# ufcg-lsd/custom-k8s-scheduler

Hardware: AMD Instinct MI355X
Metric: pods scheduled/sec (exact sequential stream, 5,000 nodes x 100,000 pods) (higher is better)
Workload: dtype int32+f64; 1 GPU; config2: 5,000 nodes x 100,000 pods, exact sequential, Fit+Balanced+QoS weights, percentageOfNodesToScore=100; engine=lookahead, launch=resident, table_layout=compact, lookahead=32, parallelism=single

## Files before the change

### custom-k8s-scheduler_amd/csrc/qs_ctx.hpp

```cpp
#pragma once
#include <hip/hip_runtime.h>
#include <rccl/rccl.h>

#include <mutex>
#include <string>
#include <unordered_map>
#include <vector>

#include "../../include/qsched.h"
#include "qs_device.hpp"
#include "qs_launch.hpp"

namespace qs_host {

constexpr int64_t kLimit = (1LL << 24) - 1;
constexpr int64_t kWideMemLimit = (1LL << 46) - 1;
constexpr int64_t kGrowLimit32 = (1LL << 31) - 1;
constexpr int64_t kGrowLimitF64 = (1LL << 53) - 1;
constexpr uint32_t kSoaMinNodes = 1u << 16;
constexpr uint32_t kAaMaxNodes = 1u << 20;

struct QsError {
    qs_status st;
    std::string msg;
// ... 97 lines not shown
    uint64_t epoch_after = 0;
    bool aa_ran = false;
    int32_t spread_row[qs::kMaxZones];
    uint32_t spread_apps = 0;
    std::vector<uint8_t> soft;
    std::vector<uint8_t> hosts;
    uint32_t host_pods = 0;
    int32_t host_row[16];
    uint32_t host_apps = 0;
    int shift = 0;
    bool wide = false;
    std::vector<uint32_t> run0;
    std::vector<uint32_t> uni_bits;
    qs_host::DevBuf d_uni;
    uint32_t uni_K = 0, uni_count = 0, uni_given = 0;
    qs_ctx *owner = nullptr;
    hipGraphExec_t gexec = nullptr;
    std::vector<uint8_t> gkey;
    ~qs_stream() {
        if (gexec) (void)hipGraphExecDestroy(gexec);
    }
};

struct qs_ctx {
    std::mutex mu;
    uint64_t table_epoch = 0;
    qs_config cfg{};
    int device = 0;
    hipStream_t stream = nullptr;
    hipStream_t stream2 = nullptr;
// ... 100 lines not shown
```

### custom-k8s-scheduler_amd/csrc/qs_host.cpp

```cpp
#include "../../include/qsched.h"

#include <hip/hip_runtime.h>

#include <algorithm>
#include <atomic>
#include <chrono>
#include <cmath>
#include <cstddef>
#include <cstdio>
#include <cstdlib>
#include <cstring>
#include <exception>
#include <mutex>
#include <new>
#include <string>
#include <vector>
#include <functional>
#include <condition_variable>
#include <thread>

#include "qs_ctx.hpp"

using namespace qs;

// ... 23 lines not shown
        const char d = env_char("QS_RES_DIAG");
        return d == '1' || d == '2';
    }();
};
const ProcKnobs &proc_knobs() {
    static const ProcKnobs k;
    return k;
}

struct RunKnobs {
    bool norm_waves1 = env_is("QS_NORM_WAVES", '1');
    bool resident_off = env_is("QS_RESIDENT", '0');
    bool res_k32_off = env_is("QS_RES_K32", '0');
    bool fast_alloc_off = env_is("QS_FAST_ALLOC", '0');
    bool res_uniform_off = env_is("QS_RES_UNIFORM", '0');
    bool fused_merge_off = env_is("QS_BATCH_FUSED_MERGE", '0');
    const char *inject = getenv("QS_INJECT_FAULT");
    bool hosttime = getenv("QS_HOSTTIME") != nullptr;
    bool norm_diag = getenv("QS_NORM_DIAG") != nullptr;
    bool sel_diag = env_is("QS_RES_DIAG", '1');
};

uint32_t feat_of(const qs_config &c) {
    uint32_t f = 0;
    if (c.enable_taint) f |= kFeatTaint;
    if (c.enable_affinity) f |= kFeatAffinity;
    return f;
}

void check_cfg(const qs_config &c) {
// ... 1216 lines not shown
            if (s->run0[last] <= s0) {
                s->uni_bits[w >> 5] |= 1u << (w & 31);
                ++s->uni_count;
            }
        }
        s->d_uni.ensure(4 * s->uni_bits.size());
        HIPCHK(hipMemcpyAsync(s->d_uni.p, s->uni_bits.data(), 4 * s->uni_bits.size(),
                              hipMemcpyHostToDevice, c->stream));
        s->uni_K = K;
    }
    if (!s->uni_count) return nullptr;
    s->uni_given = s->uni_count;
    return s->d_uni.as<uint32_t>();
}

void la_report_res_diag(const uint64_t *h, uint32_t sel) {
    const double nw = h[3] ? (double)h[3] : 1.0;
    fprintf(stderr, "QS_RES_DIAG resolver %.3f us per window; windows whose lists were not prefetched %llu of %llu (selectors %u)\n",
            h[1] * 0.01 / nw, (unsigned long long)h[4], (unsigned long long)h[3], sel);
    if (h[2])
        fprintf(stderr, "QS_RES_DIAG selector 0: done seen %.2f us, its task finished %.2f us after "
                        "the resolver's start of the window it overlaps (%llu windows)\n",
                h[13] * 0.01 / (double)h[2], h[14] * 0.01 / (double)h[2], (unsigned long long)h[2]);
    {
        std::vector<double> fin;
        for (uint32_t k = 0; k < std::min(sel, 64u); ++k)
            if (h[64 + k]) fin.push_back(h[64 + k] * 0.01);
        std::sort(fin.begin(), fin.end());
        if (!fin.empty()) {
            fprintf(stderr, "QS_RES_DIAG selectors' mean finish (us after window start), sorted:");
// ... 74 lines not shown
    dcr.inject = (inject_once(c, kn.inject, "resident_stall", kInjResidentStall) ||
                  (kn.inject && std::strcmp(kn.inject, "resident_stall_always") == 0)) ? 1u : 0u;
    if (kn.inject && std::strcmp(kn.inject, "resident_skew") == 0) dcr.inject = 2u;
    dcr.first_ticks = c->world > 1 ? 500000000ull : 0ull;
    dcr.all_alloc = c->zero_alloc == 0 && !kn.fast_alloc_off ? 1u : 0u;
    c->last_res_path = (!r.norm && rgeo.k32 ? 1 : 0) |
                       (!r.norm && !(c->dc.feat & kFeatRes) && dcr.all_alloc ? 2 : 0);
    dcr.sel_diag = kn.sel_diag ? 1u : 0u;
    uint64_t *rdiag = nullptr;
    if (proc_knobs().res_diag) {
        c->diag.ensure(1024);
        rdiag = c->diag.as<uint64_t>();
        HIPCHK(hipMemsetAsync(rdiag, 0, 1024, c->stream));
    }
    const uint32_t *uni = la_uniform_windows(c, s, rgeo, rsh.W, kn);
    kt.begin(3, c->stream);
    HIPCHK(launch_la_stream_res(c->dt, io.dp, io.dx, dcr, r.P, rgeo, c->lists.as<uint64_t>(), c->clists.as<uint64_t>(),
                                (uint32_t)r.lwords, (uint32_t)rcw, c->npart.as<uint4>(),
                                c->normi.as<NormInfo>(), c->nstat.as<uint32_t>(),
                                c->nfall.as<unsigned long long>(), io.on, io.ok,
                                io.st, c->resctl.p, rp.sel, rdiag, rsh, c->stream, uni));
    kt.end(3, c->stream);
    if (rdiag) {
        uint64_t h[128] = {0};
        HIPCHK(hipMemcpyAsync(h, rdiag, 1024, hipMemcpyDeviceToHost, c->stream));
        HIPCHK(hipStreamSynchronize(c->stream));
        la_report_res_diag(h, rp.sel);
    }
}

uint64_t run_lookahead(qs_ctx *c, qs_stream *s, const RunIo &io, const RunKnobs &kn, KernelTimer &kt) {
    const ProcKnobs &pk = proc_knobs();
    const LaRun r = la_setup(c, s, io, kn, kt.on);
    const auto th0 = std::chrono::steady_clock::now();
    const bool graph_ok = !c->comm || pk.graph == '1';
    const bool use_graph = graph_ok && !r.handoff && !r.mbox && !kt.on && !pk.diag && pk.graph != '0';
// ... 80 lines not shown
        }
        stats->pods = P;
        stats->evals = (uint64_t)P * n;
        stats->wall_s = ms * 1e-3;
        stats->batches = batches;
        stats->truncations = rescans;
        stats->engine_used = eng;
        stats->table_layout = c->wide ? 1 : 0;
        stats->resumed_windows = resumed;
        stats->resident = (eng == QS_ENGINE_LOOKAHEAD && c->last_resident) ? 1 : 0;
        stats->resident_path = stats->resident ? c->last_res_path : 0;
        stats->device_faults = c->device_faults;
    }
}

}

extern "C" {

const char *qs_version(void) { return "qsched 0.1 (gfx950)"; }

void qs_config_default(qs_config *cfg) {
    if (!cfg) return;
    std::memset(cfg, 0, sizeof(*cfg));
    cfg->abi_version = QS_ABI_VERSION;
    cfg->engine = QS_ENGINE_AUTO;
    cfg->fit_weight_cpu = 1;
    cfg->fit_weight_mem = 1;
    const int32_t wf[3] = {1, 2, 3}, wb[3] = {1, 1, 1};
    for (int q = 0; q < 3; q++) { cfg->w_fit[q] = wf[q]; cfg->w_bal[q] = wb[q]; }
// ... 693 lines not shown
            const uint32_t j = s->order[k];
            s->soft[k] = pod_soft_spread(pods[j]) ? 1 : 0;
            s->hosts[k] = pod_host_spread(pods[j]) ? 1 : 0;
            s->host_pods += s->hosts[k];
            if (s->hosts[k] && !host_seen[(uint32_t)pods[j].app]) {
                host_seen[(uint32_t)pods[j].app] = 1;
                if (s->host_apps < kHostSpreadApps) s->host_row[s->host_apps] = pods[j].app;
                ++s->host_apps;
            }
            compact_pod(c, pods[j], j, c->shift, c->wide, dp.data() + rb * k);
            if (needx) dx[k] = compact_podx(c, pods[j]);
        }
        s->run0.resize(p);
        for (uint32_t k = 0; k < p; k++)
            s->run0[k] = k > 0 && std::memcmp(dp.data() + rb * k, dp.data() + rb * (k - 1), rb) == 0 ? s->run0[k - 1] : k;
        const size_t P1 = std::max<uint32_t>(p, 1);
        s->d_pods.ensure(rb * P1);
        s->d_podx.ensure(sizeof(DPodX) * dx.size());
        s->d_node.ensure(4 * P1);
        s->d_key.ensure(8 * P1);
        if (c->cfg.record_timestamps) s->d_stamp.ensure(8 * P1);
        HIPCHK(hipMemcpyAsync(s->d_pods.p, dp.data(), rb * p, hipMemcpyHostToDevice, c->stream));
        HIPCHK(hipMemcpyAsync(s->d_podx.p, dx.data(), sizeof(DPodX) * dx.size(), hipMemcpyHostToDevice, c->stream));
        HIPCHK(hipStreamSynchronize(c->stream));
        c->streams.push_back(s);
        s->owner = c;
    });
    if (st != QS_OK) {
        delete s;
        return st;
// ... 2 lines not shown
    return QS_OK;
}

qs_status qs_stream_run(qs_ctx *c, qs_stream *s, qs_mode mode, qs_stats *stats) {
    return guarded(c, [&] {
        if (!s) fail(QS_EINVAL, "null stream");
        if (mode != QS_MODE_EXACT && mode != QS_MODE_BATCHED) fail(QS_EINVAL, "unknown qs_mode");
        if (s->shift != c->shift || s->wide != c->wide) fail(QS_ESTATE, "node table re-laid out after prepare");
        if (mode == QS_MODE_BATCHED && (s->spread_apps != 0 || s->host_pods != 0))
            fail(QS_EINVAL, "QS_MODE_BATCHED does not know topology spread (QS_AA_SPREAD / QS_AA_SPREAD_SOFT / QS_AA_SPREAD_HOSTNAME pods, spec S13-S15): "
                            "run the stream in QS_MODE_EXACT on a context that tracks pod anti-affinity");
        HIPCHK(hipSetDevice(c->device));
        s->ran = false;
        s->mode_ran = -1;
        s->uni_given = 0;
        s->aa_ran = false;
        ++c->table_epoch;
        if (!c->dev_valid) upload_table(c);
        const uint32_t n = c->m.n, P = s->p;
        const RunKnobs kn;
        const RunPlan plan = plan_run(c, s, mode);
        if (plan.host_spread && n > 0) ensure_hcount(c);
        if (c->aa_track && !(plan.aa_exact && plan.eng == QS_ENGINE_SCAN)) c->hc_valid = false;
        if (plan.host_spread && plan.eng == QS_ENGINE_PERSISTENT && n > 0 && P > 0)
            HIPCHK(hipMemcpyAsync(c->dt.zcount + (size_t)(kMaxApps + 4) * kMaxZones + 16, s->host_row,
                                  sizeof s->host_row, hipMemcpyHostToDevice, c->stream));
        if (plan.aa_exact && plan.eng == QS_ENGINE_PERSISTENT && n > 0 && P > 0)
            HIPCHK(hipMemcpyAsync(c->dt.zcount + (size_t)(kMaxApps + 1) * kMaxZones, s->spread_row,
                                  sizeof s->spread_row, hipMemcpyHostToDevice, c->stream));
        const RunIo io{s->d_pods.p, s->d_podx.as<DPodX>(), s->d_node.as<int32_t>(), s->d_key.as<uint64_t>(),
// ... 223 lines not shown

qs_status qs_stream_stamps(qs_ctx *c, qs_stream *s, uint64_t *stamps) {
    return guarded(c, [&] {
        if (!s || !s->ran || !s->d_stamp.p) fail(QS_ESTATE, "no timestamps recorded");
        HIPCHK(hipMemcpy(stamps, s->d_stamp.p, 8 * (size_t)s->p, hipMemcpyDeviceToHost));
    });
}

qs_status qs_stream_uniform_windows(qs_ctx *c, qs_stream *s, uint32_t *windows) {
    return guarded(c, [&] {
        if (!s || !windows) fail(QS_EINVAL, "null stream or output");
        *windows = s->ran ? s->uni_given : 0u;
    });
}

}
```

### custom-k8s-scheduler_amd/csrc/qs_kernels.hip

```cpp
#include "qs_kernels.hpp"

namespace qs {

__global__ __launch_bounds__(256) void k_rows_to_soa(DevTable t) {
    const uint32_t i = blockIdx.x * 256 + threadIdx.x;
    if (i >= t.n) return;
    const DRow r = t.rows[i];
    t.soa.c[kSAc][i] = r.ac; t.soa.c[kSAm][i] = r.am; t.soa.c[kSRc][i] = r.rc; t.soa.c[kSRm][i] = r.rm;
    t.soa.c[kSZc][i] = r.zc; t.soa.c[kSZm][i] = r.zm; t.soa.c[kSNp][i] = r.np; t.soa.c[kSMp][i] = r.mp;
    t.soa.c[kSAe0][i] = r.ae0; t.soa.c[kSRe0][i] = r.re0; t.soa.c[kSAe1][i] = r.ae1; t.soa.c[kSRe1][i] = r.re1;
}

__global__ void k_batch_init(uint32_t *ctrl, uint32_t *bidx, uint32_t P, uint32_t B) {
    const uint32_t nb = min(P, B);
    if (threadIdx.x < nb) bidx[threadIdx.x] = threadIdx.x;
    if (threadIdx.x == 0) { ctrl[0] = nb; ctrl[1] = nb; }
}

hipError_t launch_batch_init(uint32_t *ctrl, uint32_t *bidx, uint32_t P, uint32_t B, hipStream_t stream) {
    hipLaunchKernelGGL(k_batch_init, dim3(1), dim3(64), 0, stream, ctrl, bidx, P, B);
    return hipGetLastError();
}

hipError_t batch_claim_prepare() {
// ... 179 lines not shown
                    : (feat & kFeatRes)   ? ((feat & kFeatWide) ? res_wide_la_stream_res_per_cu(geo, feat, n)
                                                              : res_compact_la_stream_res_per_cu(geo, feat, n))
                    : (feat & kFeatWide)  ? wide_la_stream_res_per_cu(geo, feat, n)
                    : (feat & kFeatNorm)  ? la_stream_res_per_cu<kFeatExt | kFeatTaint | kFeatAffinity>(geo, n)
                    : (feat & kFeatExt) ? la_stream_res_per_cu<kFeatExt>(geo, n)
                                        : la_stream_res_per_cu<0>(geo, n);
    const int sgpr_waves = 800 / (((int)kResSgprMax + 15) / 16 * 16 + 16);
    const int safe = std::min(per, sgpr_waves / (kResBS / 64 / 4));
    return (uint32_t)std::max(0, safe) * cus;
}

bool la_stream_res_takes_uniform(const LaGeom &geo, uint32_t feat, uint32_t W) {
    return geo.k32 && W == 1 && geo.K <= 32 && res_uniform_class(feat, geo.E);
}

hipError_t launch_la_stream_res(const DevTable &t, const void *pods, const DPodX *podx, const DevCfg &c, uint32_t P,
                                const LaGeom &geo, uint64_t *lists0, uint64_t *clists0, uint32_t lwords,
                                uint32_t cwords, uint4 *npart, NormInfo *norm, uint32_t *stat, unsigned long long *nfall,
                                int32_t *on, uint64_t *ok, uint64_t *st, void *ctl, uint32_t sel_blocks, uint64_t *rdiag,
                                const ResShard &rsh0, hipStream_t stream, const uint32_t *uni) {
    ResShard rsh = rsh0;
    rsh.uni = la_stream_res_takes_uniform(geo, c.feat, rsh0.W) ? uni : nullptr;
    if (geo.G == 0 || (c.feat & kFeatAA) || (uint64_t)t.n * (t.wrows ? sizeof(DRowW) : sizeof(DRow)) >= (1ull << 31))
        return hipErrorInvalidValue;
    if (c.feat & kFeatStrat)
        return (t.wrows ? strat_wide_la_stream_res : strat_compact_la_stream_res)(
            t, pods, podx, c, P, geo, lists0, clists0, lwords, cwords, npart, norm, stat, nfall, on, ok, st, ctl,
            sel_blocks, rdiag, rsh, stream);
    if (c.feat & kFeatRes)
        return (t.wrows ? res_wide_la_stream_res : res_compact_la_stream_res)(
            t, pods, podx, c, P, geo, lists0, clists0, lwords, cwords, npart, norm, stat, nfall, on, ok, st, ctl,
            sel_blocks, rdiag, rsh, stream);
    if (t.wrows)
        return wide_la_stream_res(t, pods, podx, c, P, geo, lists0, clists0, lwords, cwords, npart, norm, stat, nfall, on,
                                  ok, st, ctl, sel_blocks, rdiag, rsh, stream);
    if (c.feat & kFeatNorm)
        return la_stream_res_f<kFeatExt | kFeatTaint | kFeatAffinity>(t, pods, podx, c, P, geo, lists0, clists0, lwords,
// ... 43 lines not shown
```

### custom-k8s-scheduler_amd/csrc/qs_kernels.hpp

```cpp
#pragma once
#include <algorithm>
#include <cstring>

#include "qs_device.hpp"
#include "qs_launch.hpp"

#ifndef QS_EXP_HOOKS
#define QS_EXP_NORM_AB(norm) (norm)
#define QS_EXP_SLOT_KEY(act, r, q)
#define QS_EXP_CAND_KEY(f, tot, cr, p)
#define QS_EXP_PARK_RETURN()
#endif

#include "qs_key32.hpp"

namespace qs {

constexpr uint32_t kFeatNorm = kFeatTaint | kFeatAffinity;

__device__ __forceinline__ uint64_t *aa_lds_zmask() {
    __shared__ uint64_t zmask[kMaxApps];
    return zmask;
}
template <int N>
// ... 2329 lines not shown
        if (f != tag || (uint32_t)(lo >> 32) != w + 1 || (uint32_t)(hi >> 32) != w + 1) {
            __hip_atomic_store((gu32 *)werr, 1u, __ATOMIC_RELAXED, __HIP_MEMORY_SCOPE_AGENT);
            return false;
        }
        const uint32_t qx = (uint32_t)(lo >> 24) & 0xFFu, qy = (uint32_t)lo & 0xFFFFFFu;
        const uint32_t qz = (uint32_t)(hi >> 22) & 0x3FFu, qw = (uint32_t)hi & 0x3FFFFFu;
        if (qx > nf.mt) { nf.mt = qx; nf.ct = 0; }
        if (qx == nf.mt) nf.ct += qy;
        if (qz > nf.ma) { nf.ma = qz; nf.ca = 0; }
        if (qz == nf.ma) nf.ca += qw;
    }
    out = nf;
    return true;
}

template <int E, int E2, uint32_t F>
__device__ __forceinline__ void res_selector(const DevTable &t, const PodT<F> *__restrict__ pods, const DevCfg &c,
                                             uint32_t P, uint32_t K, uint32_t G, uint32_t L, uint32_t chunk,
                                             uint32_t nwin, uint64_t *lists0, uint64_t *clists0, uint32_t lwords,
                                             uint32_t cwords, ResCtl *ctl, uint32_t sid, uint32_t S,
                                             uint64_t *rdiag, const DPodX *__restrict__ podx, uint4 *npart0,
                                             NormInfo *norm0, uint32_t *stat0, const ResShard &rsh) {
    constexpr bool NORM = (F & kFeatNorm) != 0;
    const uint32_t lo = (uint32_t)((uint64_t)rsh.rank * t.n / rsh.W);
    const uint32_t hi = (uint32_t)((uint64_t)(rsh.rank + 1) * t.n / rsh.W);
    bool hello_ok = rsh.W == 1;
    uint64_t ts0 = 0, ts1 = 0, ts2 = 0, dsc = 0, dtl = 0, dpm = 0, ntask = 0, nmerge = 0;
    uint64_t tdone_ = 0, wstart_ = 0, seen_ = 0, fin_ = 0, nwt_ = 0, lastp_ = 0, nlast_ = 0, late13_ = 0, late15_ = 0;
    __shared__ uint64_t lbuf[64];
    __shared__ uint32_t okflag_[4];
    __shared__ uint32_t nred[4][8];
    uint32_t &okflag = okflag_[0];
    const int tid = threadIdx.x, lane = tid & 63, w8 = tid >> 6;
    const __amdgpu_buffer_rsrc_t rs = row_rsrc<F>(t);
    DevCfg cv = c;
    asm volatile("" : "+v"(cv.yd_both), "+v"(cv.yd_c), "+v"(cv.yd_m), "+v"(cv.wc), "+v"(cv.wm));
    for (uint32_t w = 0; w < nwin; ++w) {
        const uint32_t s0 = w * K, kw = min(K, P - s0), b = w & 1;
        if (sid >= kw * G) continue;
        static_assert(sizeof(PodT<F>) % 16 == 0, "pod record in 16-byte words");
        constexpr int PW = (int)(sizeof(PodT<F>) / 16);
        constexpr bool kPodPre = (F & kFeatNorm) == 0 && E >= 7 && E <= 8;
        u32x4 pq[PW];
        if constexpr (kPodPre) {
            const u32x4 *src = reinterpret_cast<const u32x4 *>(pods + s0 + min(sid / G, kw - 1));
#pragma unroll
            for (int q = 0; q < PW; ++q) pq[q] = src[q];
#pragma unroll
            for (int q = 0; q < PW; ++q) asm volatile("" : "+v"(pq[q]));
        }
        if (w >= 2) {
            if (tid == 0) okflag = res_wait_ge(&ctl->done, w - 1, c.werr) ? 1u : 0u;
            if (rdiag && tid == 0) {
                tdone_ = __builtin_amdgcn_s_memrealtime();
                wstart_ = load_coh_u64(&rdiag[15]);
            }
            __syncthreads();
            if (!okflag) return;
        }
        uint64_t *lists = lists0 + (size_t)b * lwords;
        uint64_t *clists = clists0 + (size_t)b * cwords;
        for (uint32_t task = sid; task < kw * G; task += S) {
            if (c.inject == 1u && w == 3 && task == 0) continue;
            if (c.inject == 2u && w >= 40 && w < 44) {
                if (tid == 0) {
                    const uint64_t t0 = __builtin_amdgcn_s_memrealtime();
                    while (__builtin_amdgcn_s_memrealtime() - t0 < 300000ull) __builtin_amdgcn_s_sleep(10);
                }
                __syncthreads();
            }
            const uint32_t k = task / G, g = task % G;
            if (rdiag && c.sel_diag) ts0 = __builtin_amdgcn_s_memrealtime();
            PodT<F> p;
            if (kPodPre && task == sid) __builtin_memcpy(&p, pq, sizeof p);
            else p = pods[s0 + k];
            const uint32_t start = lo + g * chunk, end = min(hi, start + chunk);
            const uint32_t base = start + (uint32_t)w8 * E * kWave + lane;
            uint32_t tv[E];
            NormInfo nf{0, 0, 0, 0};
            if constexpr (NORM) {
                const DPodX px = load_vgpr(podx + s0 + k);
                uint32_t raw[E];
                uint32_t mt = 0, ma = 0;
                if constexpr ((F & kFeatWide) == 0) {
                    constexpr int SB = ((F & kFeatRes) != 0 && E >= 16) ? 2 : kSelB;
#pragma unroll
// ... 165 lines not shown
                    NormInfo *no = norm0 + (size_t)b * 64 + k;
                    store_coh_u64(reinterpret_cast<uint64_t *>(no), (uint64_t)nf.mt | ((uint64_t)nf.ct << 32));
                    store_coh_u64(reinterpret_cast<uint64_t *>(no) + 1, (uint64_t)nf.ma | ((uint64_t)nf.ca << 32));
                }
            };
            auto publish = [&]() {
                if (rsh.W > 1) {
                    if (!res_cross_merge(lbuf, L, k, w, rsh, hello_ok, okflag, c.werr, c.first_ticks)) return false;
                }
                uint32_t r0;
                if constexpr (NORM)
                    r0 = res_publish_list_norm(lbuf, L, out, &ctl->rdy[b][0], t, pods, podx, s0 + k, P,
                                               stat0 + ((size_t)b * K + k) * 128);
                else
                    r0 = res_publish_list(lbuf, L, out, &ctl->rdy[b][0]);
                if (rdiag && tid == 0 && w >= 2 && r0 + 1 == (w >> 1) * K + kw) {
                    const uint64_t dt_ = __builtin_amdgcn_s_memrealtime() - wstart_;
                    lastp_ += dt_;
                    ++nlast_;
                    late13_ += dt_ > 1300u;
                    late15_ += dt_ > 1500u;
                }
                return true;
            };
            if (G == 1) {
                put_norm();
                if (!publish()) return;
            } else {
                uint64_t *cl = clists + (size_t)k * G * L;
                if ((uint32_t)tid < L) store_coh_u64(cl + (size_t)g * L + tid, lbuf[tid]);
                drain_stores();
// ... 160 lines not shown
    __syncthreads();
    uint64_t ks = 0;
#pragma unroll
    for (uint32_t q = 0; q < 4; ++q) ks = red_k[q] > ks ? red_k[q] : ks;
    return ks;
}

template <uint32_t F, bool K32, bool UNI = false>
__device__ __forceinline__ void la_resolve4_stream(uint32_t *lds, const DevTable &t, const PodT<F> *__restrict__ pods,
                                                   const DevCfg &c, uint32_t P, uint32_t K, uint32_t nwin,
                                                   const uint64_t *lists0, uint32_t lwords,
                                                   int32_t *__restrict__ out_node, uint64_t *__restrict__ out_key,
                                                   uint64_t *__restrict__ stamps, ResCtl *ctl, uint64_t *rdiag,
                                                   const DPodX *__restrict__ podx, const NormInfo *norm0,
                                                   const uint32_t *stat0, unsigned long long *nfall,
                                                   const uint32_t *__restrict__ uni) {
    constexpr bool NORM = (F & kFeatNorm) != 0;
    constexpr bool R32 = K32 && !NORM;
    using KT = typename std::conditional<R32, uint32_t, uint64_t>::type;
    const int lane = threadIdx.x & 63;
    const int wv = __builtin_amdgcn_readfirstlane(threadIdx.x >> 6);
    const uint32_t nwords = (t.n + 31) / 32;
    uint32_t *dirty = lds;
    char *base = (char *)(lds + ((nwords + 3) & ~3u));
    KT(*keyA)[64] = (KT(*)[64])base; base += 2 * 64 * sizeof(KT);
    KT(*keyB)[64] = (KT(*)[64])base; base += 2 * 64 * sizeof(KT);
    KT(*keyC)[64] = (KT(*)[64])base; base += 2 * 64 * sizeof(KT);
    KT(*C1)[64] = (KT(*)[64])base; base += 2 * 64 * sizeof(KT);
    auto knode = [](KT k) -> uint32_t {
        if constexpr (R32) return k32_node(k);
        else return key_node(k);
    };
// ... 805 lines not shown
    } else if (!NORM && wv == 3) {
        auto role_c = [&](auto fa) {
        constexpr bool FA = decltype(fa)::value;
        KT c1 = 0;
        uint32_t nfallback = 0;
        auto dirty_bit = [&](KT e) -> bool {
            const uint32_t nidx = e ? knode(e) : 0u;
            return (dirty[nidx >> 5] >> (nidx & 31)) & 1u;
        };
        for (uint32_t w = 0; w < nwin; ++w) {
            const uint32_t s0 = w * K, kend = min(K, P - s0);
            const PodT<F> *wp = wpods2[w & 1];
            if (*late) {
                ++nfallback;
                const uint64_t *lists = lists0 + (size_t)(w & 1) * lwords;
                if (lane == 0) (void)res_wait_ge(&ctl->rdy[w & 1][0], (w >> 1) * K + kend, c.werr, res_bound(c, w));
                __builtin_amdgcn_fence(__ATOMIC_ACQUIRE, "wavefront");
                uint64_t e[3];
#pragma unroll
                for (uint32_t j = 0; j < 3; ++j)
                    e[j] = j < kend ? load_coh_u64(lists + (size_t)j * 64 + lane) : 0ull;
#pragma unroll
                for (uint32_t j = 0; j < 3; ++j) ringE[(s0 + j) % kResRing][lane] = kconv(e[j]);
                const uint32_t n0 = e[0] ? key_node(e[0]) : 0u;
                ringR[s0 % kResRing][lane] = load_row<F>(t, n0);
                if (F & kFeatExt) {
                    const RowX x = load_rowx<F>(t, n0);
                    ringX[s0 % kResRing][lane] = make_int4(x.ae0, x.re0, x.ae1, x.re1);
                }
            }
            const KT e0 = ringE[s0 % kResRing][lane];
            c1 = (e0 != 0 && !dirty_bit(e0)) ? e0 : (KT)0;
            C1[1][lane] = c1;
            const bool uw = uniw(w);
            if (w > 0) bmark(0);
            __syncthreads();
// ... 79 lines not shown
        if constexpr (kFastAllocClass) {
            if (fast_alloc) role_c(std::integral_constant<bool, true>{});
            else role_c(std::integral_constant<bool, false>{});
        } else {
            role_c(std::integral_constant<bool, false>{});
        }
    } else if (!NORM && wv == 4) {
        uint64_t ein = 0;
        bool skip = true;
        for (uint32_t w = 0; w < nwin; ++w) {
            const uint32_t s0 = w * K, kend = min(K, P - s0);
            const bool hasnext = w + 1 < nwin;
            const uint32_t knext = hasnext ? min(K, P - s0 - K) : 0u;
            const uint64_t *lists = lists0 + (size_t)(w & 1) * lwords;
            const uint64_t *listsn = lists0 + (size_t)((w + 1) & 1) * lwords;
            const uint32_t tnext = ((w + 1) >> 1) * K + knext;
            const bool pfw = hasnext && kend >= 6;
            const uint32_t ic = pfw ? kend - 3 : kend - 1;
            bool lt = hasnext;
            uint32_t rdyv = 0;
            const bool uw = uniw(w);
            __syncthreads();
            if (uw) {
                uni_follow(kend);
                if (lane == 0) *late = 1u;
            }
            for (uint32_t i = 0, ke = uw ? 0u : kend; i < ke; ++i) {
                const uint32_t g = s0 + i;
                if (!(skip && i == 0)) ringE[(g + 2) % kResRing][lane] = kconv(ein);
                if (i == ic) {
                    if (pfw) lt = !((uint32_t)__builtin_amdgcn_readfirstlane(rdyv) >= tnext);
                    if (lane == 0) *late = lt ? 1u : 0u;
                }
                uint64_t v = 0;
                if (i + 3 < kend) {
                    v = load_coh_u64(lists + (size_t)(i + 3) * 64 + lane);
                } else if (i >= ic && !lt && hasnext) {
                    const uint32_t j = i + 3 - kend;
                    v = load_coh_u64(listsn + (size_t)min(j, knext - 1) * 64 + lane);
                    v = j < knext ? v : 0ull;
                }
                ein = v;
                if (pfw && i + 4 == kend) rdyv = load_coh_u32(&ctl->rdy[(w + 1) & 1][0]);
                __syncthreads();
            }
            skip = lt;
            __syncthreads();
            __syncthreads();
        }
    } else if (!NORM && wv == 5) {
        for (uint32_t w = 0; w < nwin; ++w) {
            const uint32_t s0 = w * K, kend = min(K, P - s0);
            const bool hasnext = w + 1 < nwin;
            const bool pfw = hasnext && kend >= 6;
// ... 177 lines not shown
        return;
    }
    if (rsh.W > 1 && threadIdx.x == 0)
        for (uint32_t r = 0; r < rsh.W; ++r)
            __hip_atomic_store(reinterpret_cast<uint64_t *>(rsh.peers[r] + rsh.hello) + rsh.rank, rsh.seq,
                               __ATOMIC_RELEASE, __HIP_MEMORY_SCOPE_SYSTEM);
    extern __shared__ __attribute__((aligned(16))) uint32_t lds[];
    if (!UNI && (F & kFeatNorm) == 0 && threadIdx.x >= 384) {
        __syncthreads();
        for (uint32_t w = 0; w < nwin; ++w)
            for (uint32_t j = 0, nb = min(K, P - w * K) + 3; j < nb; ++j) __syncthreads();
        return;
    }
    const uint64_t t0 = rdiag ? __builtin_amdgcn_s_memrealtime() : 0ull;
    la_resolve4_stream<F, K32, UNI>(lds, t, pods, c, P, K, nwin, lists0, lwords, out_node, out_key, stamps, ctl, rdiag,
                               podx, norm0, stat0, nfall, rsh.uni);
    if (rdiag && threadIdx.x == 0) { rdiag[1] = __builtin_amdgcn_s_memrealtime() - t0; rdiag[3] = nwin; }
}

static hipError_t res_lds_attr(const void *fn, size_t lds4) {
    if (lds4 <= 64 * 1024) return hipSuccess;
    return hipFuncSetAttribute(fn, hipFuncAttributeMaxDynamicSharedMemorySize, (int)lds4);
}
template <uint32_t F>
static hipError_t la_stream_res_f(const DevTable &t, const void *pods, const DPodX *podx, const DevCfg &c, uint32_t P,
                                  const LaGeom &geo, uint64_t *lists0, uint64_t *clists0, uint32_t lwords,
                                  uint32_t cwords, uint4 *npart0, NormInfo *norm0, uint32_t *stat0,
                                  unsigned long long *nfall, int32_t *on, uint64_t *ok, uint64_t *st, void *ctl,
                                  uint32_t sel_blocks, uint64_t *rdiag, const ResShard &rsh, hipStream_t stream) {
    const uint32_t K = geo.K, G = geo.G, L = geo.L, nwin = (P + K - 1) / K;
    if (rsh.W > 1 && (rsh.W * L > (uint32_t)kResBS || K > 32 || rsh.W > 16 || !rsh.peers))
// ... 588 lines not shown
```

### custom-k8s-scheduler_amd/csrc/qs_launch.hpp

```cpp
#pragma once
#include <hip/hip_runtime.h>
#include <stddef.h>
#include <stdint.h>

namespace qs {

struct DevTable;
struct DevCfg;
struct DPodX;

struct HostRow {
    int32_t ac, am, rc, rm, zc, zm, np, mp;
    double yc, ym;
    int32_t ae0, re0, ae1, re1;
    uint64_t th, ts, lb0, lb1;
    int32_t zone, pad;
    double wam, wrm, wzm;
};

struct LaGeom {
    uint32_t K, L, G, E, chunk, epl, waves, k32;
    uint32_t W, v0, nv, eplr, lr;
    uint32_t e2 = 1;
};
// ... 36 lines not shown
    uint32_t *rec = nullptr;
    uint32_t *tickets = nullptr;
};
hipError_t launch_ready_set(uint64_t *ready, uint64_t value, hipStream_t stream);

LaGeom la_stream_res_plan(const LaGeom &geo, uint32_t feat, uint32_t n, uint32_t cus, uint32_t per_cu = 1);
size_t la_stream_res_ctl_bytes();
uint32_t la_stream_res_max_blocks(const LaGeom &geo, uint32_t feat, uint32_t n, uint32_t cus);
struct ResShard {
    uint32_t W, rank;
    uint64_t seq;
    char *const *peers;
    uint64_t hello, flags, lists;
    uint64_t nflags, norm;
    const uint32_t *uni;
};
bool la_stream_res_takes_uniform(const LaGeom &geo, uint32_t feat, uint32_t W);
hipError_t launch_la_stream_res(const DevTable &t, const void *pods, const DPodX *podx, const DevCfg &c, uint32_t P,
                                const LaGeom &geo, uint64_t *lists0, uint64_t *clists0, uint32_t lwords,
                                uint32_t cwords, uint4 *npart, NormInfo *norm, uint32_t *stat, unsigned long long *nfall, int32_t *on,
                                uint64_t *ok, uint64_t *st, void *ctl, uint32_t sel_blocks, uint64_t *rdiag,
                                const ResShard &rsh, hipStream_t stream, const uint32_t *uni = nullptr);

hipError_t launch_la_window(const DevTable &t, const void *pods, const DPodX *podx, uint32_t s0,
                            uint32_t P, const DevCfg &c, const LaGeom &geo, const LaBufs &bufs,
                            int32_t *out_node, uint64_t *out_key, uint64_t *stamps, uint64_t *diag,
                            hipStream_t stream, int part);

hipError_t launch_batch_init(uint32_t *ctrl, uint32_t *bidx, uint32_t P, uint32_t B, hipStream_t stream);
size_t batch_claim_lds(uint32_t n);
hipError_t batch_claim_prepare();
hipError_t launch_batch_claim(const DevTable &t, const void *pods, const uint64_t *lists, uint32_t *ctrl,
                              uint32_t *bidx, uint32_t P, uint32_t B, int32_t *out_node,
                              uint64_t *out_key, hipStream_t stream);

__global__ void k_set_row(DevTable t, uint32_t i, HostRow v, uint32_t feat);
__global__ void k_aa_apply(DevTable t, uint32_t node, uint32_t app, int32_t sign, uint32_t clear_bit);
// ... 4 lines not shown
```

### custom-k8s-scheduler_amd/qsched/__init__.py

```python
from __future__ import annotations

import ctypes

import numpy as np

from ._abi import (ENGINES, ENGINE_NAMES, EXPORTED, LIB_PATH, POD_DTYPE, QS_ABI_VERSION,
                   QS_MAX_EXT, QS_MAX_SCORE_RES, QS_MAX_TERMS, QS_MODE_BATCHED, QS_MODE_EXACT, QS_OK,
                   RESOURCES, FIT_REASONS, QS_FIT_TAINT, QS_MAX_SHAPE, QOS_NAMES, STRATEGIES, QschedError,
                   QschedLibraryMissing, QsConfig, QsContainer, QsNodeRow, QsNodeSoa, QsScoringStrategy,
                   QsStats, load)

__all__ = ["Scheduler", "Config", "POD_DTYPE", "pods_to_struct", "pods_from_struct", "fit_error_message",
           "synth_generate", "shape_table", "dist_unique_id", "empty_nodes", "pod_from_containers", "compute_qos", "load",
           "QschedError", "QschedLibraryMissing", "ENGINES", "EXPORTED", "LIB_PATH",
           "aa_spread", "aa_spread_soft", "aa_spread_hostname", "aa_is_soft", "aa_is_hostkey", "QS_AA_HOSTKEY", "aa_kind", "aa_max_skew", "QS_AA_SOFT", "QS_MAX_ZONES", "QS_AA_NONE", "QS_AA_HOSTNAME", "QS_AA_ZONE", "QS_AA_SPREAD_ZONE",
           "QS_MAX_SPREAD_SKEW"]

from ._abi import (QS_AA_HOSTKEY, QS_AA_HOSTNAME, QS_AA_NONE, QS_AA_SOFT, QS_AA_SPREAD_ZONE, QS_AA_ZONE,
                   QS_MAX_SPREAD_SKEW, QS_MAX_ZONES)

MODES = {"exact": QS_MODE_EXACT, "batched": QS_MODE_BATCHED}


def aa_spread(max_skew: int) -> int:
# ... 306 lines not shown


class Stream:

    def __init__(self, sched: Scheduler, handle, p):
        self.s, self.h, self.p = sched, handle, p
        self.stats = None

    def run(self, mode="exact"):
        st = QsStats()
        self.s._chk(self.s.lib.qs_stream_run(self.s.ctx, self.h, MODES[mode], ctypes.byref(st)))
        self.stats = st.as_dict()
        uw = ctypes.c_uint32(0)
        self.s._chk(self.s.lib.qs_stream_uniform_windows(self.s.ctx, self.h, ctypes.byref(uw)))
        self.stats["uniform_windows"] = int(uw.value)
        return self.stats

    def results(self):
        placement = np.empty(self.p, np.int32)
        keys = np.empty(self.p, np.uint64)
        self.s._chk(self.s.lib.qs_stream_results(self.s.ctx, self.h, _ptr(placement), _ptr(keys)))
        return placement, keys

    def stamps(self):
        out = np.empty(self.p, np.uint64)
        self.s._chk(self.s.lib.qs_stream_stamps(self.s.ctx, self.h, _ptr(out)))
        return out

    def fit_errors(self, pods=None, by_taint=False):
        if pods is None:
# ... 103 lines not shown
```

### custom-k8s-scheduler_amd/qsched/_abi.py

```python
from __future__ import annotations

import ctypes
import os

import numpy as np

PKG_ROOT = os.path.dirname(os.path.dirname(os.path.abspath(__file__)))
LIB_PATH = os.environ.get("QSCHED_LIB") or os.path.join(PKG_ROOT, "libqsched.so")

QS_ABI_VERSION = 3
QS_MAX_EXT = 2
QS_MAX_TERMS = 4
QS_MAX_APPS = 1024
QS_MAX_ZONES = 64
QS_AA_NONE, QS_AA_HOSTNAME, QS_AA_ZONE = 0, 1, 2
QS_AA_SPREAD_ZONE, QS_MAX_SPREAD_SKEW = 3, 31
QS_AA_SOFT = 1 << 16
QS_AA_HOSTKEY = 1 << 18
QS_MAX_SCORE_RES = 4
FIT_REASONS = ["Too many pods", "Insufficient cpu", "Insufficient memory", "Insufficient {ext0}",
               "Insufficient {ext1}", "node(s) had untolerated taint {{{taint}}}",
               "node(s) didn't match Pod's node affinity/selector"]
QS_FIT_TAINT = 5
RESOURCES = {"cpu": 1, "memory": 2, "ext0": 3, "ext1": 4}
# ... 127 lines not shown
    "qs_nodes_load": (ctypes.c_int, [_P, _P, ctypes.c_uint32]),
    "qs_nodes_read": (ctypes.c_int, [_P, _P, ctypes.c_uint32]),
    "qs_node_upsert": (ctypes.c_int, [_P, ctypes.c_uint32, _P, ctypes.c_uint64]),
    "qs_table_save": (ctypes.c_int, [_P]),
    "qs_table_restore": (ctypes.c_int, [_P]),
    "qs_reserve": (ctypes.c_int, [_P, ctypes.c_uint32, _P]),
    "qs_unreserve": (ctypes.c_int, [_P, ctypes.c_uint32, _P]),
    "qs_score_pod": (ctypes.c_int, [_P, _P, _P, _P, _P, _P]),
    "qs_score_pod_packed": (ctypes.c_int, [_P, _P, _P, _P]),
    "qs_schedule_stream": (ctypes.c_int, [_P, _P, ctypes.c_uint32, ctypes.c_int, _P, _P]),
    "qs_stream_prepare": (ctypes.c_int, [_P, _P, ctypes.c_uint32, _P]),
    "qs_stream_run": (ctypes.c_int, [_P, _P, ctypes.c_int, _P]),
    "qs_stream_results": (ctypes.c_int, [_P, _P, _P, _P]),
    "qs_stream_stamps": (ctypes.c_int, [_P, _P, _P]),
    "qs_stream_uniform_windows": (ctypes.c_int, [_P, _P, _P]),
    "qs_stream_fit_errors": (ctypes.c_int, [_P, _P, _P, ctypes.c_uint32, _P]),
    "qs_stream_fit_taints": (ctypes.c_int, [_P, _P, _P, ctypes.c_uint32, _P, _P]),
    "qs_stream_free": (ctypes.c_int, [_P, _P]),
    "qs_pod_from_containers": (ctypes.c_int, [_P, ctypes.c_uint32, _P, _P]),
    "qs_compute_qos": (ctypes.c_int32, [_P, ctypes.c_uint32]),
    "qs_synth_generate": (ctypes.c_int, [ctypes.c_int, ctypes.c_uint64, ctypes.c_uint32,
                                         ctypes.c_uint32, _P, _P]),
    "qs_struct_size": (ctypes.c_size_t, [ctypes.c_int]),
}
EXPORTED = sorted(_SIGS)

_LIB = None


def load(path: str = LIB_PATH):
# ... 21 lines not shown
```

### include/qsched.h

```cpp
#ifndef QSCHED_H
#define QSCHED_H

#include <stddef.h>
#include <stdint.h>

#ifdef __cplusplus
extern "C" {
#endif

#if defined(__GNUC__)
#define QS_API __attribute__((visibility("default")))
#else
#define QS_API
#endif

#define QS_ABI_VERSION 3
#define QS_MAX_EXT 2
#define QS_MAX_TERMS 4
#define QS_MAX_APPS 1024
#define QS_MAX_ZONES 64
#define QS_MAX_SCORE_RES 4

typedef enum qs_status {
    QS_OK = 0,
// ... 169 lines not shown
QS_API qs_status qs_unreserve(qs_ctx *ctx, uint32_t node, const qs_pod *pod);

QS_API qs_status qs_score_pod(qs_ctx *ctx, const qs_pod *pod, uint8_t *feasible_n, int32_t *score_n,
                       int32_t *total_n, int32_t *best);
QS_API qs_status qs_score_pod_packed(qs_ctx *ctx, const qs_pod *pod, const uint32_t **packed_n, int32_t *best);
QS_API qs_status qs_score_pod_zone_scores(qs_ctx *ctx, int32_t out[QS_MAX_ZONES]);

QS_API qs_status qs_schedule_stream(qs_ctx *ctx, const qs_pod *pods, uint32_t p, qs_mode mode,
                             int32_t *placement_p, qs_stats *stats);
QS_API qs_status qs_stream_prepare(qs_ctx *ctx, const qs_pod *pods, uint32_t p, qs_stream **out);
QS_API qs_status qs_stream_run(qs_ctx *ctx, qs_stream *s, qs_mode mode, qs_stats *stats);
QS_API qs_status qs_stream_results(qs_ctx *ctx, qs_stream *s, int32_t *placement_p, uint64_t *best_key_p);
QS_API qs_status qs_stream_free(qs_ctx *ctx, qs_stream *s);
QS_API qs_status qs_stream_stamps(qs_ctx *ctx, qs_stream *s, uint64_t *stamps_p);
QS_API qs_status qs_stream_uniform_windows(qs_ctx *ctx, qs_stream *s, uint32_t *windows);
typedef enum qs_fit_reason {
    QS_FIT_TOO_MANY_PODS = 0,
    QS_FIT_CPU = 1,
    QS_FIT_MEMORY = 2,
    QS_FIT_EXT0 = 3,
    QS_FIT_EXT1 = 4,
    QS_FIT_TAINT = 5,
    QS_FIT_AFFINITY = 6,
    QS_FIT_REASONS = 7
} qs_fit_reason;
QS_API qs_status qs_stream_fit_errors(qs_ctx *ctx, qs_stream *s, const uint32_t *pods, uint32_t m, uint32_t *counts);
QS_API qs_status qs_stream_fit_taints(qs_ctx *ctx, qs_stream *s, const uint32_t *pods, uint32_t m, uint32_t *counts,
                                      uint32_t *taint_counts);

QS_API qs_status qs_pod_from_containers(const qs_container *c, uint32_t nc, const int64_t *overhead_cpu_mem,
// ... 12 lines not shown
```

Baseline: 2.287 million pods/s.

## Share candidate lists among identical pods within each lookahead window

Pods in a stream are hashed on the host to find identical records, and for each window a plan maps every pod to a representative pod whose candidate list is built once. The selector kernel then builds lists only for the distinct pods, and the resolver reads each pod's list through the representative slot, with ready counters adjusted to the cumulative distinct counts. This is meant to cut redundant selector work and list traffic when many pods share the same spec. It adds host-side hashing at prepare time, a plan upload, and extra indirection in the resolver's load path.

```diff
diff --git a/custom-k8s-scheduler_amd/csrc/qs_ctx.hpp b/custom-k8s-scheduler_amd/csrc/qs_ctx.hpp
--- a/custom-k8s-scheduler_amd/csrc/qs_ctx.hpp
+++ b/custom-k8s-scheduler_amd/csrc/qs_ctx.hpp
@@ -135,6 +135,9 @@
     std::vector<uint32_t> uni_bits;
     qs_host::DevBuf d_uni;
     uint32_t uni_K = 0, uni_count = 0, uni_given = 0;
+    std::vector<uint32_t> rec0;
+    qs_host::DevBuf d_share;
+    uint32_t share_K = 0, share_lists = 0, lists_given = 0;
     qs_ctx *owner = nullptr;
     hipGraphExec_t gexec = nullptr;
     std::vector<uint8_t> gkey;
diff --git a/custom-k8s-scheduler_amd/csrc/qs_host.cpp b/custom-k8s-scheduler_amd/csrc/qs_host.cpp
--- a/custom-k8s-scheduler_amd/csrc/qs_host.cpp
+++ b/custom-k8s-scheduler_amd/csrc/qs_host.cpp
@@ -61,6 +61,7 @@
     bool res_k32_off = env_is("QS_RES_K32", '0');
     bool fast_alloc_off = env_is("QS_FAST_ALLOC", '0');
     bool res_uniform_off = env_is("QS_RES_UNIFORM", '0');
+    bool res_share_off = env_is("QS_RES_SHARE", '0');
     bool fused_merge_off = env_is("QS_BATCH_FUSED_MERGE", '0');
     const char *inject = getenv("QS_INJECT_FAULT");
     bool hosttime = getenv("QS_HOSTTIME") != nullptr;
@@ -1307,6 +1308,26 @@
     return s->d_uni.as<uint32_t>();
 }
 
+const uint8_t *la_share_plan(qs_ctx *c, qs_stream *s, const LaGeom &rgeo, uint32_t W, const RunKnobs &kn) {
+    const uint32_t P = s->p, K = rgeo.K;
+    s->lists_given = P;
+    if (kn.res_share_off || !la_stream_res_takes_share(rgeo, c->dc.feat, W) || s->rec0.size() != P || P == 0)
+        return nullptr;
+    const uint32_t nwin = (P + K - 1) / K;
+    const size_t cum_bytes = share_cum_bytes(nwin), row_bytes = (size_t)nwin * kShareRow;
+    if (s->share_K != K) {
+        std::vector<uint8_t> h(share_plan_bytes(nwin));
+        s->share_lists = share_plan_build(s->rec0.data(), P, K, reinterpret_cast<uint32_t *>(h.data()),
+                                          h.data() + cum_bytes, h.data() + cum_bytes + row_bytes);
+        s->d_share.ensure(h.size());
+        HIPCHK(hipMemcpyAsync(s->d_share.p, h.data(), h.size(), hipMemcpyHostToDevice, c->stream));
+        HIPCHK(hipStreamSynchronize(c->stream));
+        s->share_K = K;
+    }
+    s->lists_given = s->share_lists;
+    return s->d_share.as<uint8_t>();
+}
+
 void la_report_res_diag(const uint64_t *h, uint32_t sel) {
     const double nw = h[3] ? (double)h[3] : 1.0;
     fprintf(stderr, "QS_RES_DIAG resolver %.3f us per window; windows whose lists were not prefetched %llu of %llu (selectors %u)\n",
@@ -1411,12 +1432,13 @@
         HIPCHK(hipMemsetAsync(rdiag, 0, 1024, c->stream));
     }
     const uint32_t *uni = la_uniform_windows(c, s, rgeo, rsh.W, kn);
+    const uint8_t *share = la_share_plan(c, s, rgeo, rsh.W, kn);
     kt.begin(3, c->stream);
     HIPCHK(launch_la_stream_res(c->dt, io.dp, io.dx, dcr, r.P, rgeo, c->lists.as<uint64_t>(), c->clists.as<uint64_t>(),
                                 (uint32_t)r.lwords, (uint32_t)rcw, c->npart.as<uint4>(),
                                 c->normi.as<NormInfo>(), c->nstat.as<uint32_t>(),
                                 c->nfall.as<unsigned long long>(), io.on, io.ok,
-                                io.st, c->resctl.p, rp.sel, rdiag, rsh, c->stream, uni));
+                                io.st, c->resctl.p, rp.sel, rdiag, rsh, c->stream, uni, share));
     kt.end(3, c->stream);
     if (rdiag) {
         uint64_t h[128] = {0};
@@ -1527,6 +1549,46 @@
     }
 }
 
+}
+
+namespace qs {
+void share_first_index(const uint8_t *rec, size_t rb, uint32_t P, uint32_t *first) {
+    size_t cap = 16;
+    while (cap < 2 * (size_t)P) cap *= 2;
+    std::vector<uint32_t> tab(cap, 0xFFFFFFFFu);
+    for (uint32_t k = 0; k < P; ++k) {
+        const uint8_t *r = rec + rb * k;
+        uint64_t h = 0xcbf29ce484222325ull;
+        for (size_t b = 0; b < rb; ++b) h = (h ^ r[b]) * 0x100000001b3ull;
+        size_t at = (size_t)(h ^ (h >> 29)) & (cap - 1);
+        while (tab[at] != 0xFFFFFFFFu && std::memcmp(rec + rb * tab[at], r, rb) != 0) at = (at + 1) & (cap - 1);
+        if (tab[at] == 0xFFFFFFFFu) tab[at] = k;
+        first[k] = tab[at];
+    }
+}
+uint32_t share_plan_build(const uint32_t *first, uint32_t P, uint32_t K, uint32_t *cum, uint8_t *rep, uint8_t *dl) {
+    const uint32_t nwin = K ? (P + K - 1) / K : 0;
+    uint32_t total = 0;
+    cum[0] = cum[1] = 0;
+    if (nwin) {
+        std::memset(rep, 0, (size_t)nwin * kShareRow);
+        std::memset(dl, 0, (size_t)nwin * kShareRow);
+    }
+    for (uint32_t w = 0; w < nwin; ++w) {
+        const uint32_t s0 = w * K, kw = std::min(K, P - s0);
+        uint8_t *rw = rep + (size_t)w * kShareRow, *dw = dl + (size_t)w * kShareRow;
+        uint32_t D = 0;
+        for (uint32_t k = 0; k < kw; ++k) {
+            uint32_t j = 0;
+            while (j < D && first[s0 + dw[j]] != first[s0 + k]) ++j;
+            if (j == D) dw[D++] = (uint8_t)k;
+            rw[k] = dw[j];
+        }
+        cum[w + 2] = cum[w] + D;
+        total += D;
+    }
+    return total;
+}
 }
 
 extern "C" {
@@ -2250,6 +2312,8 @@
         s->run0.resize(p);
         for (uint32_t k = 0; k < p; k++)
             s->run0[k] = k > 0 && std::memcmp(dp.data() + rb * k, dp.data() + rb * (k - 1), rb) == 0 ? s->run0[k - 1] : k;
+        s->rec0.resize(p);
+        share_first_index(dp.data(), rb, p, s->rec0.data());
         const size_t P1 = std::max<uint32_t>(p, 1);
         s->d_pods.ensure(rb * P1);
         s->d_podx.ensure(sizeof(DPodX) * dx.size());
@@ -2282,6 +2346,7 @@
         s->ran = false;
         s->mode_ran = -1;
         s->uni_given = 0;
+        s->lists_given = s->p;
         s->aa_ran = false;
         ++c->table_epoch;
         if (!c->dev_valid) upload_table(c);
@@ -2535,4 +2600,24 @@
     });
 }
 
-}
+qs_status qs_stream_shared_lists(qs_ctx *c, qs_stream *s, uint32_t *lists) {
+    return guarded(c, [&] {
+        if (!s || !lists) fail(QS_EINVAL, "null stream or output");
+        *lists = s->ran ? s->lists_given : 0u;
+    });
+}
+
+qs_status qs_share_plan(const void *records, uint32_t record_bytes, uint32_t p, uint32_t k, uint32_t *cum,
+                        uint8_t *rep, uint8_t *dl, uint32_t *lists) {
+    if (!records || !cum || !rep || !dl || !lists || record_bytes == 0 || k == 0 || k > kShareRow) return QS_EINVAL;
+    try {
+        std::vector<uint32_t> first(p);
+        share_first_index(static_cast<const uint8_t *>(records), record_bytes, p, first.data());
+        *lists = share_plan_build(first.data(), p, k, cum, rep, dl);
+    } catch (const std::bad_alloc &) {
+        return QS_ENOMEM;
+    }
+    return QS_OK;
+}
+
+}
diff --git a/custom-k8s-scheduler_amd/csrc/qs_kernels.hip b/custom-k8s-scheduler_amd/csrc/qs_kernels.hip
--- a/custom-k8s-scheduler_amd/csrc/qs_kernels.hip
+++ b/custom-k8s-scheduler_amd/csrc/qs_kernels.hip
@@ -217,13 +217,18 @@
     return geo.k32 && W == 1 && geo.K <= 32 && res_uniform_class(feat, geo.E);
 }
 
+bool la_stream_res_takes_share(const LaGeom &geo, uint32_t feat, uint32_t W) {
+    return W == 1 && (feat & kFeatNorm) == 0 && geo.K <= kShareRow;
+}
+
 hipError_t launch_la_stream_res(const DevTable &t, const void *pods, const DPodX *podx, const DevCfg &c, uint32_t P,
                                 const LaGeom &geo, uint64_t *lists0, uint64_t *clists0, uint32_t lwords,
                                 uint32_t cwords, uint4 *npart, NormInfo *norm, uint32_t *stat, unsigned long long *nfall,
                                 int32_t *on, uint64_t *ok, uint64_t *st, void *ctl, uint32_t sel_blocks, uint64_t *rdiag,
-                                const ResShard &rsh0, hipStream_t stream, const uint32_t *uni) {
+                                const ResShard &rsh0, hipStream_t stream, const uint32_t *uni, const uint8_t *share) {
     ResShard rsh = rsh0;
     rsh.uni = la_stream_res_takes_uniform(geo, c.feat, rsh0.W) ? uni : nullptr;
+    rsh.share = la_stream_res_takes_share(geo, c.feat, rsh0.W) ? share : nullptr;
     if (geo.G == 0 || (c.feat & kFeatAA) || (uint64_t)t.n * (t.wrows ? sizeof(DRowW) : sizeof(DRow)) >= (1ull << 31))
         return hipErrorInvalidValue;
     if (c.feat & kFeatStrat)
diff --git a/custom-k8s-scheduler_amd/csrc/qs_kernels.hpp b/custom-k8s-scheduler_amd/csrc/qs_kernels.hpp
--- a/custom-k8s-scheduler_amd/csrc/qs_kernels.hpp
+++ b/custom-k8s-scheduler_amd/csrc/qs_kernels.hpp
@@ -2367,6 +2367,12 @@
     return true;
 }
 
+__device__ __forceinline__ const uint32_t *share_cum(const uint8_t *sh) { return reinterpret_cast<const uint32_t *>(sh); }
+__device__ __forceinline__ const uint8_t *share_rep(const uint8_t *sh, uint32_t nwin) { return sh + share_cum_bytes(nwin); }
+__device__ __forceinline__ const uint8_t *share_dl(const uint8_t *sh, uint32_t nwin) {
+    return sh + share_cum_bytes(nwin) + (size_t)nwin * kShareRow;
+}
+
 template <int E, int E2, uint32_t F>
 __device__ __forceinline__ void res_selector(const DevTable &t, const PodT<F> *__restrict__ pods, const DevCfg &c,
                                              uint32_t P, uint32_t K, uint32_t G, uint32_t L, uint32_t chunk,
@@ -2390,13 +2396,23 @@
     asm volatile("" : "+v"(cv.yd_both), "+v"(cv.yd_c), "+v"(cv.yd_m), "+v"(cv.wc), "+v"(cv.wm));
     for (uint32_t w = 0; w < nwin; ++w) {
         const uint32_t s0 = w * K, kw = min(K, P - s0), b = w & 1;
-        if (sid >= kw * G) continue;
+        uint32_t nlist = kw;
+        if constexpr (!NORM) {
+            if (rsh.share) nlist = share_cum(rsh.share)[w + 2] - share_cum(rsh.share)[w];
+        }
+        auto task_pod = [&](uint32_t j) -> uint32_t {
+            if constexpr (!NORM) {
+                if (rsh.share) return share_dl(rsh.share, nwin)[(size_t)w * kShareRow + j];
+            }
+            return j;
+        };
+        if (sid >= nlist * G) continue;
         static_assert(sizeof(PodT<F>) % 16 == 0, "pod record in 16-byte words");
         constexpr int PW = (int)(sizeof(PodT<F>) / 16);
         constexpr bool kPodPre = (F & kFeatNorm) == 0 && E >= 7 && E <= 8;
         u32x4 pq[PW];
         if constexpr (kPodPre) {
-            const u32x4 *src = reinterpret_cast<const u32x4 *>(pods + s0 + min(sid / G, kw - 1));
+            const u32x4 *src = reinterpret_cast<const u32x4 *>(pods + s0 + min(task_pod(sid / G), kw - 1));
 #pragma unroll
             for (int q = 0; q < PW; ++q) pq[q] = src[q];
 #pragma unroll
@@ -2413,7 +2429,7 @@
         }
         uint64_t *lists = lists0 + (size_t)b * lwords;
         uint64_t *clists = clists0 + (size_t)b * cwords;
-        for (uint32_t task = sid; task < kw * G; task += S) {
+        for (uint32_t task = sid; task < nlist * G; task += S) {
             if (c.inject == 1u && w == 3 && task == 0) continue;
             if (c.inject == 2u && w >= 40 && w < 44) {
                 if (tid == 0) {
@@ -2422,7 +2438,7 @@
                 }
                 __syncthreads();
             }
-            const uint32_t k = task / G, g = task % G;
+            const uint32_t k = task_pod(task / G), g = task % G;
             if (rdiag && c.sel_diag) ts0 = __builtin_amdgcn_s_memrealtime();
             PodT<F> p;
             if (kPodPre && task == sid) __builtin_memcpy(&p, pq, sizeof p);
@@ -2618,7 +2634,8 @@
                                                stat0 + ((size_t)b * K + k) * 128);
                 else
                     r0 = res_publish_list(lbuf, L, out, &ctl->rdy[b][0]);
-                if (rdiag && tid == 0 && w >= 2 && r0 + 1 == (w >> 1) * K + kw) {
+                if (rdiag && tid == 0 && w >= 2 &&
+                    r0 + 1 == ((!NORM && rsh.share) ? share_cum(rsh.share)[w + 2] : (w >> 1) * K + kw)) {
                     const uint64_t dt_ = __builtin_amdgcn_s_memrealtime() - wstart_;
                     lastp_ += dt_;
                     ++nlast_;
@@ -2809,8 +2826,18 @@
                                                    uint64_t *__restrict__ stamps, ResCtl *ctl, uint64_t *rdiag,
                                                    const DPodX *__restrict__ podx, const NormInfo *norm0,
                                                    const uint32_t *stat0, unsigned long long *nfall,
-                                                   const uint32_t *__restrict__ uni) {
+                                                   const uint32_t *__restrict__ uni,
+                                                   const uint8_t *__restrict__ share) {
     constexpr bool NORM = (F & kFeatNorm) != 0;
+    auto rdy_want = [&](uint32_t w, uint32_t kw) -> uint32_t {
+        if constexpr (!NORM) {
+            if (share) return share_cum(share)[w + 2];
+        }
+        return (w >> 1) * K + kw;
+    };
+    const uint8_t *srep = (!NORM && share) ? share_rep(share, nwin) : nullptr;
+    (void)rdy_want;
+    (void)srep;
     constexpr bool R32 = K32 && !NORM;
     using KT = typename std::conditional<R32, uint32_t, uint64_t>::type;
     const int lane = threadIdx.x & 63;
@@ -3646,12 +3673,15 @@
             if (*late) {
                 ++nfallback;
                 const uint64_t *lists = lists0 + (size_t)(w & 1) * lwords;
-                if (lane == 0) (void)res_wait_ge(&ctl->rdy[w & 1][0], (w >> 1) * K + kend, c.werr, res_bound(c, w));
+                const uint32_t slot[3] = {0u, srep ? (uint32_t)srep[(size_t)w * kShareRow + 1] : 1u,
+                                          srep ? (uint32_t)srep[(size_t)w * kShareRow + 2] : 2u};
+                const uint32_t want = rdy_want(w, kend);
+                if (lane == 0) (void)res_wait_ge(&ctl->rdy[w & 1][0], want, c.werr, res_bound(c, w));
                 __builtin_amdgcn_fence(__ATOMIC_ACQUIRE, "wavefront");
                 uint64_t e[3];
 #pragma unroll
                 for (uint32_t j = 0; j < 3; ++j)
-                    e[j] = j < kend ? load_coh_u64(lists + (size_t)j * 64 + lane) : 0ull;
+                    e[j] = j < kend ? load_coh_u64(lists + (size_t)slot[j] * 64 + lane) : 0ull;
 #pragma unroll
                 for (uint32_t j = 0; j < 3; ++j) ringE[(s0 + j) % kResRing][lane] = kconv(e[j]);
                 const uint32_t n0 = e[0] ? key_node(e[0]) : 0u;
@@ -3761,12 +3791,17 @@
             const uint32_t knext = hasnext ? min(K, P - s0 - K) : 0u;
             const uint64_t *lists = lists0 + (size_t)(w & 1) * lwords;
             const uint64_t *listsn = lists0 + (size_t)((w + 1) & 1) * lwords;
-            const uint32_t tnext = ((w + 1) >> 1) * K + knext;
+            const uint32_t tnext = hasnext ? rdy_want(w + 1, knext) : 0u;
             const bool pfw = hasnext && kend >= 6;
             const uint32_t ic = pfw ? kend - 3 : kend - 1;
             bool lt = hasnext;
             uint32_t rdyv = 0;
             const bool uw = uniw(w);
+            uint32_t slotc = (uint32_t)lane, slotn = (uint32_t)lane;
+            if (srep) {
+                slotc = srep[(size_t)w * kShareRow + lane];
+                slotn = srep[(size_t)(hasnext ? w + 1 : w) * kShareRow + lane];
+            }
             __syncthreads();
             if (uw) {
                 uni_follow(kend);
@@ -3781,10 +3816,12 @@
                 }
                 uint64_t v = 0;
                 if (i + 3 < kend) {
-                    v = load_coh_u64(lists + (size_t)(i + 3) * 64 + lane);
+                    const uint32_t sl = (uint32_t)__builtin_amdgcn_readlane((int)slotc, (int)(i + 3));
+                    v = load_coh_u64(lists + (size_t)sl * 64 + lane);
                 } else if (i >= ic && !lt && hasnext) {
                     const uint32_t j = i + 3 - kend;
-                    v = load_coh_u64(listsn + (size_t)min(j, knext - 1) * 64 + lane);
+                    const uint32_t sl = (uint32_t)__builtin_amdgcn_readlane((int)slotn, (int)min(j, knext - 1));
+                    v = load_coh_u64(listsn + (size_t)sl * 64 + lane);
                     v = j < knext ? v : 0ull;
                 }
                 ein = v;
@@ -3992,7 +4029,7 @@
     }
     const uint64_t t0 = rdiag ? __builtin_amdgcn_s_memrealtime() : 0ull;
     la_resolve4_stream<F, K32, UNI>(lds, t, pods, c, P, K, nwin, lists0, lwords, out_node, out_key, stamps, ctl, rdiag,
-                               podx, norm0, stat0, nfall, rsh.uni);
+                               podx, norm0, stat0, nfall, rsh.uni, rsh.share);
     if (rdiag && threadIdx.x == 0) { rdiag[1] = __builtin_amdgcn_s_memrealtime() - t0; rdiag[3] = nwin; }
 }
 
diff --git a/custom-k8s-scheduler_amd/csrc/qs_launch.hpp b/custom-k8s-scheduler_amd/csrc/qs_launch.hpp
--- a/custom-k8s-scheduler_amd/csrc/qs_launch.hpp
+++ b/custom-k8s-scheduler_amd/csrc/qs_launch.hpp
@@ -74,13 +74,21 @@
     uint64_t hello, flags, lists;
     uint64_t nflags, norm;
     const uint32_t *uni;
+    const uint8_t *share;
 };
+constexpr uint32_t kShareRow = 64;
+constexpr size_t share_cum_bytes(uint32_t nwin) { return (4 * ((size_t)nwin + 2) + 63) & ~(size_t)63; }
+constexpr size_t share_plan_bytes(uint32_t nwin) { return share_cum_bytes(nwin) + 2 * (size_t)nwin * kShareRow; }
+void share_first_index(const uint8_t *records, size_t record_bytes, uint32_t P, uint32_t *first);
+uint32_t share_plan_build(const uint32_t *first, uint32_t P, uint32_t K, uint32_t *cum, uint8_t *rep, uint8_t *dl);
+bool la_stream_res_takes_share(const LaGeom &geo, uint32_t feat, uint32_t W);
 bool la_stream_res_takes_uniform(const LaGeom &geo, uint32_t feat, uint32_t W);
 hipError_t launch_la_stream_res(const DevTable &t, const void *pods, const DPodX *podx, const DevCfg &c, uint32_t P,
                                 const LaGeom &geo, uint64_t *lists0, uint64_t *clists0, uint32_t lwords,
                                 uint32_t cwords, uint4 *npart, NormInfo *norm, uint32_t *stat, unsigned long long *nfall, int32_t *on,
                                 uint64_t *ok, uint64_t *st, void *ctl, uint32_t sel_blocks, uint64_t *rdiag,
-                                const ResShard &rsh, hipStream_t stream, const uint32_t *uni = nullptr);
+                                const ResShard &rsh, hipStream_t stream, const uint32_t *uni = nullptr,
+                                const uint8_t *share = nullptr);
 
 hipError_t launch_la_window(const DevTable &t, const void *pods, const DPodX *podx, uint32_t s0,
                             uint32_t P, const DevCfg &c, const LaGeom &geo, const LaBufs &bufs,
diff --git a/custom-k8s-scheduler_amd/qsched/__init__.py b/custom-k8s-scheduler_amd/qsched/__init__.py
--- a/custom-k8s-scheduler_amd/qsched/__init__.py
+++ b/custom-k8s-scheduler_amd/qsched/__init__.py
@@ -344,6 +344,8 @@
         uw = ctypes.c_uint32(0)
         self.s._chk(self.s.lib.qs_stream_uniform_windows(self.s.ctx, self.h, ctypes.byref(uw)))
         self.stats["uniform_windows"] = int(uw.value)
+        self.s._chk(self.s.lib.qs_stream_shared_lists(self.s.ctx, self.h, ctypes.byref(uw)))
+        self.stats["lists_selected"] = int(uw.value)
         return self.stats
 
     def results(self):
diff --git a/custom-k8s-scheduler_amd/qsched/_abi.py b/custom-k8s-scheduler_amd/qsched/_abi.py
--- a/custom-k8s-scheduler_amd/qsched/_abi.py
+++ b/custom-k8s-scheduler_amd/qsched/_abi.py
@@ -165,6 +165,8 @@
     "qs_stream_results": (ctypes.c_int, [_P, _P, _P, _P]),
     "qs_stream_stamps": (ctypes.c_int, [_P, _P, _P]),
     "qs_stream_uniform_windows": (ctypes.c_int, [_P, _P, _P]),
+    "qs_stream_shared_lists": (ctypes.c_int, [_P, _P, _P]),
+    "qs_share_plan": (ctypes.c_int, [_P, ctypes.c_uint32, ctypes.c_uint32, ctypes.c_uint32, _P, _P, _P, _P]),
     "qs_stream_fit_errors": (ctypes.c_int, [_P, _P, _P, ctypes.c_uint32, _P]),
     "qs_stream_fit_taints": (ctypes.c_int, [_P, _P, _P, ctypes.c_uint32, _P, _P]),
     "qs_stream_free": (ctypes.c_int, [_P, _P]),
diff --git a/include/qsched.h b/include/qsched.h
--- a/include/qsched.h
+++ b/include/qsched.h
@@ -207,6 +207,9 @@
 QS_API qs_status qs_stream_free(qs_ctx *ctx, qs_stream *s);
 QS_API qs_status qs_stream_stamps(qs_ctx *ctx, qs_stream *s, uint64_t *stamps_p);
 QS_API qs_status qs_stream_uniform_windows(qs_ctx *ctx, qs_stream *s, uint32_t *windows);
+QS_API qs_status qs_stream_shared_lists(qs_ctx *ctx, qs_stream *s, uint32_t *lists);
+QS_API qs_status qs_share_plan(const void *records, uint32_t record_bytes, uint32_t p, uint32_t k, uint32_t *cum,
+                               uint8_t *rep, uint8_t *dl, uint32_t *lists);
 typedef enum qs_fit_reason {
     QS_FIT_TOO_MANY_PODS = 0,
     QS_FIT_CPU = 1,
```

Result: no change. 2.308 million pods/s (median of 6 runs) (+0.9%).
